# yassouali/pytorch-segmentation

Hardware: NVIDIA H100
Metric: images/sec DeepLabV3+/ResNet101 513x513 train step (fwd+CE+bwd+SGD) (higher is better)
Workload: dtype bf16

## Files before the change

include/seg_b200.h:

```cpp
#ifndef SEG_B200_H
#define SEG_B200_H

#include <stdint.h>

#ifdef __cplusplus
extern "C" {
#endif

#define SEG_DT_BF16 0
#define SEG_DT_F32 1

#define SEG_IMPL_AUTO 0
#define SEG_IMPL_SIMT 1
#define SEG_IMPL_TC 2

typedef struct seg_conv_desc {
  int32_t N, H, W, C;
  int32_t K;
  int32_t R, S;
  int32_t stride, pad, dil;
  int32_t P, Q;
  int32_t ldx;
  int32_t ldy;
} seg_conv_desc;

typedef struct seg_sync_desc {
  void* const* peers;
  int32_t rank, world, n_max;
  int64_t timeout_clocks;
  int32_t mode;
} seg_sync_desc;

const char* seg_last_error(void);
int seg_version(void);
int seg_device_ok(void);
int64_t seg_launch_count(void);
void seg_launch_count_reset(void);

int seg_conv2d_fwd(const seg_conv_desc* d, const void* x, const void* w_packed, void* y, int y_dtype,
                   const float* bias, float beta, double* stats, const seg_sync_desc* sync, void* sync_ticket,
                   int impl, void* stream);
int seg_conv2d_dgrad(const seg_conv_desc* d, const void* dy, const void* w_packed, void* dx, float beta,
                     int impl, void* stream);
int64_t seg_conv2d_wgrad_workspace_floats(const seg_conv_desc* d, int impl);
int seg_conv2d_wgrad(const seg_conv_desc* d, const void* dy, const void* x, float* dw_packed, float* workspace, int impl,
                     void* stream);

int64_t seg_dwconv_scratch_floats(int C);
int seg_dwconv3x3_fwd(const seg_conv_desc* d, const void* x, const float* w9, void* y, double* stats,
                      const seg_sync_desc* sync, void* sync_ticket, void* stream);
int seg_dwconv3x3_bwd_data(const seg_conv_desc* d, const void* dy, const float* w9, void* dx, float beta, void* stream);
int seg_dwconv3x3_bwd_weight(const seg_conv_desc* d, const void* dy, const void* x, float* dw9, float beta,
                             float* scratch, void* stream);
int seg_dw_pack_weight(const float* w_c133, float* w9, int C, void* stream);
int seg_dw_unpack_wgrad(const float* g9, float* g_c133, int C, float beta, void* stream);

int seg_pack_weight(const float* w_oihw, void* w_packed, int K, int C, int R, int S, int Cpad, void* stream);
int seg_unpack_wgrad(const float* dw_packed, float* g_oihw, int K, int C, int R, int S, int Cpad, float beta,
                     void* stream);
int seg_pack_entry_bytes(void);
int seg_pack_weights_batched(const void* table, int n, int64_t total, void* stream);
int seg_unpack_wgrads_batched(const void* table, int n, int64_t total, float beta, void* stream);
int seg_im2col(const seg_conv_desc* d, const void* x, int x_nchw_f32, void* col, int Kpad, void* stream);

int seg_bn_stats(const void* x, int64_t M, int C, int ldx, double* stats, const seg_sync_desc* sync, void* sync_ticket,
                 void* stream);
int seg_bn_finalize(const double* stats, double count, int C, const float* gamma, const float* beta, float eps,
                    float momentum, int clamp_eps, float* running_mean, float* running_var, float* scale_shift,
                    float* save_mean_istd, void* stream);
// ... 141 lines not shown
```

pytorch-segmentation_b200/csrc/seg_api.cu:

```cuda
#include <stdarg.h>
#include "seg_common.cuh"
#include "seg_sync.cuh"

namespace seg {

static thread_local char g_err[1024] = "";
std::atomic<long long> g_launches{0};

void set_error(const char* fmt, ...) {
  va_list ap;
  va_start(ap, fmt);
  vsnprintf(g_err, sizeof(g_err), fmt, ap);
  va_end(ap);
}

namespace tc {
bool supported(const seg_conv_desc* d);
int conv_fwd(const seg_conv_desc* d, const void* x, const void* w, void* y, int y_dtype, const float* bias, float beta,
             double* stats, unsigned* stat_ticket, const SyncDesc* sync, cudaStream_t stream);
int conv_dgrad(const seg_conv_desc* d, const void* dy, const void* w, void* dx, float beta, cudaStream_t stream);
int conv_wgrad(const seg_conv_desc* d, const void* dy, const void* x, float* dw, float* ws, cudaStream_t stream);
int64_t wgrad_workspace_floats(const seg_conv_desc* d);
}
namespace simt {
int conv_fwd(const seg_conv_desc* d, const void* x, const void* w, void* y, int y_dtype, const float* bias, float beta,
             double* stats, unsigned* stat_ticket, const seg_sync_desc* sync, cudaStream_t stream);
int conv_dgrad(const seg_conv_desc* d, const void* dy, const void* w, void* dx, float beta, cudaStream_t stream);
int conv_wgrad(const seg_conv_desc* d, const void* dy, const void* x, float* dw, cudaStream_t stream);
}

static int check_desc(const seg_conv_desc* d) {
  SEG_REQUIRE(d != nullptr, "null conv descriptor");
  SEG_REQUIRE(d->N > 0 && d->H > 0 && d->W > 0 && d->C > 0 && d->K > 0 && d->R > 0 && d->S > 0, "bad conv dims");
  SEG_REQUIRE(d->stride >= 1 && d->dil >= 1 && d->pad >= 0, "bad conv stride/dil/pad");
  const int P = (d->H + 2 * d->pad - d->dil * (d->R - 1) - 1) / d->stride + 1;
  const int Q = (d->W + 2 * d->pad - d->dil * (d->S - 1) - 1) / d->stride + 1;
  SEG_REQUIRE(P == d->P && Q == d->Q, "conv output size mismatch: expected %dx%d got %dx%d", P, Q, d->P, d->Q);
  SEG_REQUIRE(d->ldx >= d->C && d->ldy >= d->K, "conv pitch smaller than channel count");
  return 0;
}

static bool tma_base_ok(const void* p) { return (reinterpret_cast<uintptr_t>(p) & 15) == 0; }

}
// ... 40 lines not shown
    return tc::conv_fwd(d, x, w_packed, y, y_dtype, bias, beta, stats, tk, sync ? &sd : nullptr, ST(stream));
  }
  return simt::conv_fwd(d, x, w_packed, y, y_dtype, bias, beta, stats, tk, sync, ST(stream));
}

int seg_conv2d_dgrad(const seg_conv_desc* d, const void* dy, const void* w_packed, void* dx, float beta, int impl,
                     void* stream) {
  if (check_desc(d)) return 1;
  const bool tc_ok = tc::supported(d) && d->ldy % 8 == 0 && tma_base_ok(dy) && tma_base_ok(w_packed);
  if (impl == SEG_IMPL_TC || (impl == SEG_IMPL_AUTO && tc_ok))
    return tc::conv_dgrad(d, dy, w_packed, dx, beta, ST(stream));
  return simt::conv_dgrad(d, dy, w_packed, dx, beta, ST(stream));
}

static bool wgrad_on_tc(const seg_conv_desc* d, int impl) {
  return impl == SEG_IMPL_TC || (impl == SEG_IMPL_AUTO && tc::supported(d) && d->ldy % 8 == 0);
}

int64_t seg_conv2d_wgrad_workspace_floats(const seg_conv_desc* d, int impl) {
  if (check_desc(d)) return -1;
  return wgrad_on_tc(d, impl) ? tc::wgrad_workspace_floats(d) : 0;
}

int seg_conv2d_wgrad(const seg_conv_desc* d, const void* dy, const void* x, float* dw_packed, float* workspace, int impl,
                     void* stream) {
  if (check_desc(d)) return 1;
  if (wgrad_on_tc(d, impl) && (impl == SEG_IMPL_TC || (tma_base_ok(dy) && tma_base_ok(x))))
    return tc::conv_wgrad(d, dy, x, dw_packed, workspace, ST(stream));
  return simt::conv_wgrad(d, dy, x, dw_packed, ST(stream));
}

}
```

pytorch-segmentation_b200/csrc/seg_conv_tc.cu:

```cuda
#include <cuda.h>
#include <mutex>
#include <stdlib.h>
#include "seg_common.cuh"
#include "seg_ptx.cuh"
#include "seg_sync.cuh"

namespace seg {
namespace tc {

using namespace ptx;

constexpr int BM = 128;
constexpr int BK = 64;
constexpr int A_BYTES = BM * 128;
constexpr int KIND_KK = 0, KIND_KM = 1;
constexpr int NTHREADS = 384;
constexpr int NCONS = 256;
constexpr int MAXT = 49;

constexpr int BAR_CONSUMERS = 1;
constexpr int BAR_ORDER = 2;
constexpr int BAR_WG = 4;

struct TcParams {
// ... 3 lines not shown
  int Ncols;
  int taps;
  int kchunks;
  int stride;
  int lower_h, lower_w;
  int PQ, Q;
  int x_im2col;
  int brows_per_tap;
  short tap_wt[MAXT];
  short tap_oh[MAXT];
  short tap_ow[MAXT];
  void* out;
  long long ldo;
  int out_dtype;
  float beta;
  const float* bias;
  double* stats;
  int stat_rows;
  unsigned* stat_ticket;
  SyncDesc sync;
  int out_strided, out_H, out_W, osy, osx, opy, opx;
  int n_tiles, tiles;
  int kblocks_total, kblocks_per_split;
  float* dw;
  int dw_K, dw_C;
  float* ws;
};

__device__ __forceinline__ void row_to_coords(int m, int PQ, int Q, int stride, int lower_h, int lower_w, int& n, int& h,
                                              int& w) {
  n = m / PQ;
  int rem = m - n * PQ;
  int pp = rem / Q;
  int qq = rem - pp * Q;
  h = lower_h + pp * stride;
  w = lower_w + qq * stride;
}

template <int BN, int TA, int TB>
__device__ __forceinline__ void wgmma_tile(float* acc, uint64_t adesc, uint64_t bdesc, uint32_t accumulate) {
  if constexpr (BN == 64) wgmma_m64n64k16<TA, TB>(acc, adesc, bdesc, accumulate);
  else if constexpr (BN == 128) wgmma_m64n128k16<TA, TB>(acc, adesc, bdesc, accumulate);
  else wgmma_m64n256k16<TA, TB>(acc, adesc, bdesc, accumulate);
}

template <int BN, int KIND>
// ... 274 lines not shown

template <int BN>
struct Cfg {
  static constexpr int B_BYTES = BN * 128;
  static constexpr int STAGE_BYTES = A_BYTES + B_BYTES;
  static constexpr int STAGES = BN == 64 ? 6 : (BN == 128 ? 5 : 4);
  static constexpr int SMEM = STAGES * STAGE_BYTES + 1024  + 256 ;
  static_assert(STAGES * STAGE_BYTES >= BM * BN * 4, "staging tile must fit in the pipeline ring");
  static_assert(SMEM <= 227 * 1024, "shared memory per block");
};

template <int BN>
__global__ void __launch_bounds__(NTHREADS, 1) conv_gemm_wgrad(const __grid_constant__ TcParams p) {
  using C = Cfg<BN>;
  constexpr int STAGES = C::STAGES;
  extern __shared__ uint8_t smem_raw[];
  const uint32_t raw_addr = smem_u32(smem_raw);
  const uint32_t smem0 = (raw_addr + 1023u) & ~1023u;
  uint8_t* smem_gen = smem_raw + (smem0 - raw_addr);
  const uint32_t bar0 = smem0 + STAGES * C::STAGE_BYTES;
  auto full_bar = [&](int s) { return bar0 + 8u * s; };
  auto empty_bar = [&](int s) { return bar0 + 8u * (STAGES + s); };

  const int m0 = blockIdx.x * BM;
  const int n0 = blockIdx.y * BN;

  const int tap_mm = blockIdx.z % p.taps;
  const int split = blockIdx.z / p.taps;
  const int kb_begin = split * p.kblocks_per_split;
  const int kb_end = min(kb_begin + p.kblocks_per_split, p.kblocks_total);
  const int num_iters = max(kb_end - kb_begin, 0);

  if (threadIdx.x == 0) {
    prefetch_tmap(&p.mapA);
    prefetch_tmap(&p.mapB);
    for (int s = 0; s < STAGES; ++s) {
      mbar_init(full_bar(s), 1);
      mbar_init(empty_bar(s), 8);
    }
    fence_mbar_init();
  }
  __syncthreads();
  pdl_wait();

  if (threadIdx.x < 128) {
    if (threadIdx.x == 0 && num_iters > 0) {
      const uint16_t oh = (uint16_t)p.tap_oh[tap_mm], ow = (uint16_t)p.tap_ow[tap_mm];
      int it = 0;
      for (int kb = kb_begin; kb < kb_end; ++kb, ++it) {
        const int st = it % STAGES;
        const uint32_t ph = (it / STAGES) & 1;
        mbar_wait_nocall(empty_bar(st), ph ^ 1u);
        const uint32_t a_dst = smem0 + st * C::STAGE_BYTES;
        const uint32_t b_dst = a_dst + A_BYTES;
        const int pix0 = kb * BK;
        mbar_arrive_expect_tx(full_bar(st), C::STAGE_BYTES);
        tma_load_2d(a_dst, &p.mapA, full_bar(st), m0, pix0);
        tma_load_2d(a_dst + 8192, &p.mapA, full_bar(st), m0 + 64, pix0);
        if (p.x_im2col) {
          int n_img, h0, w0;
          row_to_coords(pix0, p.PQ, p.Q, p.stride, p.lower_h, p.lower_w, n_img, h0, w0);
#pragma unroll
          for (int j = 0; j < BN / 64; ++j)
            tma_load_im2col_4d(b_dst + j * 8192, &p.mapB, full_bar(st), n0 + j * 64, w0, h0, n_img, ow, oh);
        } else {
#pragma unroll
          for (int j = 0; j < BN / 64; ++j) tma_load_2d(b_dst + j * 8192, &p.mapB, full_bar(st), n0 + j * 64, pix0);
        }
      }
    }
    return;
  }

  if (num_iters == 0) return;
  const int ctid = threadIdx.x - 128;
  const int cw = ctid >> 7;
  const int warp = (ctid >> 5) & 3, lane = ctid & 31;
  float acc[BN / 2];
#pragma unroll
  for (int i = 0; i < BN / 2; ++i) acc[i] = 0.f;
  for (int it = 0; it < num_iters; ++it) {
    const int st = it % STAGES;
    mbar_wait_nocall(full_bar(st), (it / STAGES) & 1);
    const uint32_t a_addr = smem0 + st * C::STAGE_BYTES + cw * 8192;
    const uint32_t b_addr = smem0 + st * C::STAGE_BYTES + A_BYTES;
    const uint64_t adesc0 = make_smem_desc_sw128(a_addr, 8192, 1024);
    const uint64_t bdesc0 = make_smem_desc_sw128(b_addr, 8192, 1024);
    wgmma_fence();
#pragma unroll
    for (int k = 0; k < BK / 16; ++k)
      wgmma_tile<BN, 1, 1>(acc, adesc0 + (uint64_t)(k * 2048 >> 4), bdesc0 + (uint64_t)(k * 2048 >> 4), 1u);
    wgmma_commit();
    wgmma_wait<1>();
    __syncwarp();
    if (it > 0 && lane == 0) mbar_arrive(empty_bar((it - 1) % STAGES));
  }
  wgmma_wait<0>();
  named_sync(BAR_CONSUMERS, NCONS);

  uint8_t* stage = smem_gen;
  const int ncols_tile = min(BN, p.Ncols - n0);
  stage_acc<BN>(acc, nullptr, stage, cw * 64, warp, lane, nullptr, true);
  named_sync(BAR_CONSUMERS, NCONS);

  const int CPR = BN * 4 / 16;
  const int swz = (CPR >= 32 ? 31 : CPR - 1);
  float* base = p.ws ? p.ws + (size_t)split * p.taps * p.dw_K * p.dw_C : p.dw;
  for (int idx = ctid; idx < BM * CPR; idx += NCONS) {
    const int tr = idx / CPR, c16 = idx - tr * CPR;
    const int row = m0 + tr, col0 = c16 * 4;
    if (row >= p.M || col0 >= ncols_tile) continue;
    const float4 v = *reinterpret_cast<const float4*>(stage + (size_t)tr * (BN * 4) + ((c16 ^ (tr & swz)) << 4));
    float* dst = base + ((size_t)tap_mm * p.dw_K + row) * p.dw_C + n0 + col0;
    const bool vec = col0 + 4 <= ncols_tile && ((reinterpret_cast<uintptr_t>(dst) & 15) == 0);
    const float a[4] = {v.x, v.y, v.z, v.w};
    if (p.ws) {
      if (vec)
        *reinterpret_cast<float4*>(dst) = v;
      else
        for (int i = 0; i < 4; ++i)
          if (col0 + i < ncols_tile) dst[i] = a[i];
    } else if (vec) {
      asm volatile("red.global.add.v4.f32 [%0], {%1, %2, %3, %4};" ::"l"(dst), "f"(v.x), "f"(v.y), "f"(v.z), "f"(v.w)
                   : "memory");
    } else {
      for (int i = 0; i < 4; ++i)
        if (col0 + i < ncols_tile) atomicAdd(dst + i, a[i]);
    }
  }
}

typedef CUresult (*EncodeTiledFn)(CUtensorMap*, CUtensorMapDataType, cuuint32_t, void*, const cuuint64_t*,
                                  const cuuint64_t*, const cuuint32_t*, const cuuint32_t*, CUtensorMapInterleave,
                                  CUtensorMapSwizzle, CUtensorMapL2promotion, CUtensorMapFloatOOBfill);
typedef CUresult (*EncodeIm2colFn)(CUtensorMap*, CUtensorMapDataType, cuuint32_t, void*, const cuuint64_t*,
                                   const cuuint64_t*, const int*, const int*, cuuint32_t, cuuint32_t,
                                   const cuuint32_t*, CUtensorMapInterleave, CUtensorMapSwizzle,
                                   CUtensorMapL2promotion, CUtensorMapFloatOOBfill);
static EncodeTiledFn g_encode_tiled = nullptr;
static EncodeIm2colFn g_encode_im2col = nullptr;
static int g_driver_version = 0;

static int resolve_driver() {
  static std::once_flag once;
  static int status = 0;
  std::call_once(once, [] {
    void* f1 = nullptr;
    void* f2 = nullptr;
    cudaDriverEntryPointQueryResult q;
    if (cudaGetDriverEntryPoint("cuTensorMapEncodeTiled", &f1, cudaEnableDefault, &q) != cudaSuccess || !f1) status = 1;
    if (cudaGetDriverEntryPoint("cuTensorMapEncodeIm2col", &f2, cudaEnableDefault, &q) != cudaSuccess || !f2) status = 1;
// ... 252 lines not shown
    dw[i] += acc;
  }
}

static void wgrad_plan(const seg_conv_desc* d, int& bn, int& splits, int& kblocks_per_split) {
  const bool wide = d->R * d->S >= 9 && d->C >= 256 && d->C % 256 == 0;
  bn = (d->C <= 64) ? 64 : (wide ? 256 : 128);
  const int kblocks_total = (int)ceil_div64((int64_t)d->N * d->P * d->Q, BK);
  const int tiles = ceil_div(d->K, BM) * ceil_div(d->C, bn) * d->R * d->S;
  splits = max(1, num_sms() / tiles);
  splits = min(splits, kblocks_total);
  splits = min(splits, 1024);
  kblocks_per_split = ceil_div(kblocks_total, splits);
  splits = ceil_div(kblocks_total, kblocks_per_split);
}

int64_t wgrad_workspace_floats(const seg_conv_desc* d) {
  if (!supported(d)) return 0;
  int bn, splits, kps;
  wgrad_plan(d, bn, splits, kps);
  return splits > 1 ? (int64_t)splits * d->R * d->S * d->K * d->C : 0;
}

int conv_wgrad(const seg_conv_desc* d, const void* dy, const void* x, float* dw, float* ws, cudaStream_t stream) {
  SEG_REQUIRE(supported(d) && d->ldy % 8 == 0, "wgmma conv wgrad: unsupported shape");
  TcParams p;
  memset(&p, 0, sizeof(p));
  const int64_t npix = (int64_t)d->N * d->P * d->Q;
  SEG_REQUIRE(npix < (1ll << 31), "too many pixels");
  p.M = d->K;
  p.Ncols = d->C;
  p.taps = d->R * d->S;
  for (int t = 0; t < p.taps; ++t) {
    p.tap_wt[t] = (short)t;
    p.tap_oh[t] = (short)((t / d->S) * d->dil);
    p.tap_ow[t] = (short)((t % d->S) * d->dil);
  }
  p.stride = d->stride;
  p.lower_h = p.lower_w = -d->pad;
  p.PQ = d->P * d->Q;
  p.Q = d->Q;
  p.dw = dw;
  p.dw_K = d->K;
  p.dw_C = d->C;
  p.kblocks_total = (int)ceil_div64(npix, BK);
  int bn, splits;
  wgrad_plan(d, bn, splits, p.kblocks_per_split);
  SEG_REQUIRE(splits == 1 || ws != nullptr, "wgmma conv wgrad: %d k-splits need the workspace (seg_conv2d_wgrad_workspace_floats)", splits);
  SEG_REQUIRE((int64_t)(splits - 1) * p.kblocks_per_split < p.kblocks_total, "wgmma conv wgrad: split %d has no k-blocks", splits - 1);
  if (splits > 1) p.ws = ws;
  if (make_map_2d(&p.mapA, dy, npix, d->K, d->ldy, 64)) return 1;
  if (is_pointwise(d)) {
    p.x_im2col = 0;
    if (make_map_2d(&p.mapB, x, npix, d->C, d->ldx, 64)) return 1;
  } else {
    p.x_im2col = 1;
    const int upper = d->pad - (d->R - 1) * d->dil;
    if (make_map_im2col(&p.mapB, x, d->N, d->H, d->W, d->C, d->ldx, -d->pad, -d->pad, upper, upper, d->stride, 64)) return 1;
  }
  SEG_REQUIRE((unsigned)(p.taps * splits) <= 65535u, "wgrad grid.z too large");
  dim3 grid((unsigned)ceil_div(d->K, BM), (unsigned)ceil_div(d->C, bn), (unsigned)(p.taps * splits));
  if (launch_wgrad_bn(bn, p, grid, stream)) return 1;
  if (splits == 1) return 0;
  const int64_t n = (int64_t)p.taps * d->K * d->C;
  wgrad_split_reduce_kernel<<<(unsigned)std::min<int64_t>(ceil_div64(n, 256), (int64_t)num_sms() * 8), 256, 0, stream>>>(ws, splits, n, dw);
  return check_launch("wgrad_split_reduce");
}

}
}
```

pytorch-segmentation_b200/seg_b200/engine.py:

```python
import torch

from . import ops
from .lib import IMPL_AUTO

BN_EPS = 1e-5
BN_MOM = 0.1
FUSED_BWD_MAX_BYTES = 24 << 20
ACT_DTYPE = torch.bfloat16


class Act:
    __slots__ = ("t", "grad", "needs_grad", "_written")

    def __init__(self, t, needs_grad=True):
        self.t = t
        self.grad = None
        self.needs_grad = needs_grad
        self._written = False

    @property
    def shape(self):
        return self.t.shape

    def grad_target(self):
        if self.grad is None:
            self.grad = torch.empty(self.t.shape, dtype=ACT_DTYPE, device=self.t.device)
        if not self._written:
            self._written = True
            return self.grad, 0.0
        return self.grad, 1.0

# ... 68 lines not shown
                 step_ctr=None, arena_floats=0, owner=None):
        self.training = training
        self.record = training if record is None else record
        self.back = []
        self.back_params = {}
        self.grads = grads if grads is not None else {}
        self.touched = set()
        self.impl = impl
        self.dropout = dropout
        self.seed = seed
        self.sync = sync
        self.step_ctr = step_ctr
        self.packed_override = {}
        self.dw_buffers = {}
        self.clamp_eps = clamp_eps
        self._drop_ctr = 0
        self._pushed = set()
        self.bn_modules = []
        self.owner = owner
        self._arena_hint = int(arena_floats)
        self._arena = None
        self._arena_off = 0
        self.arena_used = 0

    def sync_active(self):
        s = self.sync
        return s is not None and (s.world > 1 or getattr(s, "force", False))

    def sync_fused(self):
        return self.sync_active() and getattr(self.sync, "fused", False)

    def zalloc(self, n, device):
        n_al = (int(n) + 31) // 32 * 32
        if self._arena is None or self._arena_off + n_al > self._arena.numel() or self._arena.device != device:
            size = max(self._arena_hint if self._arena is None else 0, n_al, 1 << 20)
            self._arena = torch.zeros(size, dtype=torch.float32, device=device)
            self._arena_off = 0
        v = self._arena[self._arena_off:self._arena_off + int(n)]
        self._arena_off += n_al
        self.arena_used += n_al
        return v

    def zalloc64(self, n, device):
        return self.zalloc(2 * int(n), device).view(torch.float64)

    def _param_grad(self, p, value_fn):
        if not p.requires_grad:
            return
        self.touched.add(p)
        if p in self.grads:
            value_fn(self.grads[p], 1.0)
        else:
            g = torch.empty(p.shape, dtype=torch.float32, device=p.device)
            value_fn(g, 0.0)
            self.grads[p] = g

    def _push_back(self, fn, params=()):
        if params:
            self.back_params[len(self.back)] = tuple(p for p in params if p is not None)
        self.back.append(fn)

    def backward(self, after=None):
        for i in range(len(self.back) - 1, -1, -1):
            self.back[i]()
            if after is not None:
                after(i)
        if self.owner is not None and self.arena_used:
            self.owner._arena_floats = self.arena_used
        self.back = []

    def conv(self, x, spec, out=None, out_dtype=None, want_stats=False):
        wp = self.packed_override.get(spec)
        if wp is None:
            wp = spec.packed()
        bias = spec.m.bias
        stats = None
        if out_dtype is None:
            out_dtype = ACT_DTYPE
        want = want_stats and self.training
        sync = tk = None
        if want:
            stats = self.zalloc64(2 * spec.K, wp.device)
            if self.sync_fused():
                sync, tk = self.sync, self.zalloc(1, wp.device)
        if spec.explicit:
            nchw = not isinstance(x, Act)
            src = x if nchw else x.t
            col = ops.im2col(src, spec.R, spec.S, spec.stride, spec.pad, spec.dil, spec.kpad, nchw_f32=nchw)
            y = ops.conv2d_fwd(col, wp, spec.K, 1, 1, out=out, out_dtype=out_dtype, bias=bias.detach() if bias is not None else None,
                               stats=stats, impl=self.impl, sync=sync, sync_ticket=tk)
            xin, geo = col, (1, 1, 1, 0, 1)
        else:
            y = ops.conv2d_fwd(x.t, wp, spec.K, spec.R, spec.S, spec.stride, spec.pad, spec.dil, out=out, out_dtype=out_dtype,
                               bias=bias.detach() if bias is not None else None, stats=stats, impl=self.impl, sync=sync, sync_ticket=tk)
            xin, geo = x.t, (spec.R, spec.S, spec.stride, spec.pad, spec.dil)
        ya = Act(y)
        if sync is not None:
            self._pushed.add(stats.data_ptr())
        if self.record:
            def bwd():
                dy = ya.grad
                if dy is None:
                    return
                R, S, stride, pad, dil = geo
                if spec.m.weight.requires_grad and spec in self.dw_buffers:
                    ops.conv2d_wgrad(dy, xin, R, S, stride, pad, dil, out=self.dw_buffers[spec], impl=self.impl)
                    self.touched.add(spec.m.weight)
                elif spec.m.weight.requires_grad:
                    dwp = ops.conv2d_wgrad(dy, xin, R, S, stride, pad, dil, impl=self.impl)
                    if spec.explicit:
                        def fill(g, beta):
                            full = dwp[0, :, : spec.R * spec.S * spec.C].reshape(spec.K, spec.R, spec.S, spec.C).permute(0, 3, 1, 2)
                            if beta:
                                g.add_(full)
                            else:
                                g.copy_(full)
                    else:
                        def fill(g, beta):
                            ops.unpack_wgrad(dwp, tuple(spec.m.weight.shape), beta=beta, out=g)
                    self._param_grad(spec.m.weight, fill)
                if bias is not None and bias.requires_grad:
                    cpad = ops.ld(dy)
                    wide = dy if dy.shape[-1] % 8 == 0 else dy.as_strided(dy.shape[:-1] + (cpad,), dy.stride(), dy.storage_offset())
                    s = ops.bn_stats(wide)[: spec.K].float()
                    self._param_grad(bias, lambda g, beta: g.add_(s) if beta else g.copy_(s))
                if (not spec.explicit) and isinstance(x, Act) and x.needs_grad:
                    gx, beta = x.grad_target()
                    ops.conv2d_dgrad(dy, wp, tuple(x.t.shape), R, S, stride, pad, dil, out=gx, beta=beta, impl=self.impl)
                ya.grad = None
            self._push_back(bwd, (spec.m.weight, bias))
        return ya, stats

    def dwconv(self, x, spec, want_stats=False):
        w9 = spec.packed()
        stats = self.zalloc64(2 * spec.C, w9.device) if (want_stats and self.training) else None
        sync = self.sync if (stats is not None and self.sync_fused()) else None
        y = ops.dwconv_fwd(x.t, w9, spec.stride, spec.pad, spec.dil, stats=stats, sync=sync,
                           sync_ticket=self.zalloc(1, w9.device) if sync is not None else None)
        if sync is not None:
            self._pushed.add(stats.data_ptr())
        ya = Act(y)
        if self.record:
            def bwd():
                dy = ya.grad
                if dy is None:
                    return
                if spec.m.weight.requires_grad:
                    g9 = ops.dwconv_bwd_weight(dy, x.t, spec.stride, spec.pad, spec.dil)
                    self._param_grad(spec.m.weight, lambda g, beta: ops.dw_unpack_wgrad(g9, g, beta))
                if x.needs_grad:
                    gx, beta = x.grad_target()
                    ops.dwconv_bwd_data(dy, w9, tuple(x.t.shape), spec.stride, spec.pad, spec.dil, out=gx, beta=beta)
                ya.grad = None
            self._push_back(bwd, (spec.m.weight,))
# ... 197 lines not shown
```

pytorch-segmentation_b200/seg_b200/lib.py:

```python
import ctypes
import os
from ctypes import POINTER, Structure, c_char_p, c_double, c_float, c_int, c_int32, c_int64, c_uint8, c_uint32, c_uint64, c_void_p

import torch

_HERE = os.path.dirname(os.path.abspath(__file__))
LIB_PATH = os.path.join(os.path.dirname(_HERE), "libseg_b200.so")

DT_BF16, DT_F32 = 0, 1
IMPL_AUTO, IMPL_SIMT, IMPL_TC = 0, 1, 2
LOSS_CE, LOSS_WCE, LOSS_FOCAL = 0, 1, 2


class SyncDesc(Structure):

    _fields_ = [("peers", c_void_p), ("rank", c_int32), ("world", c_int32), ("n_max", c_int32), ("timeout_clocks", c_int64),
                ("mode", c_int32)]


class ConvDesc(Structure):

    _fields_ = [(n, c_int32) for n in ("N", "H", "W", "C", "K", "R", "S", "stride", "pad", "dil", "P", "Q", "ldx", "ldy")]


def conv_out_size(size, k, stride, pad, dil):
    return (size + 2 * pad - dil * (k - 1) - 1) // stride + 1


def make_conv_desc(N, H, W, C, K, R, S, stride, pad, dil, ldx=None, ldy=None):
    P = conv_out_size(H, R, stride, pad, dil)
    Q = conv_out_size(W, S, stride, pad, dil)
    return ConvDesc(N, H, W, C, K, R, S, stride, pad, dil, P, Q, ldx if ldx is not None else C, ldy if ldy is not None else K)


_SIGS = {
    "seg_last_error": (c_char_p, []),
    "seg_version": (c_int, []),
    "seg_device_ok": (c_int, []),
    "seg_launch_count": (c_int64, []),
    "seg_launch_count_reset": (None, []),
    "seg_conv2d_fwd": (c_int, [POINTER(ConvDesc), c_void_p, c_void_p, c_void_p, c_int, c_void_p, c_float, c_void_p, c_void_p, c_void_p, c_int, c_void_p]),
    "seg_conv2d_dgrad": (c_int, [POINTER(ConvDesc), c_void_p, c_void_p, c_void_p, c_float, c_int, c_void_p]),
    "seg_conv2d_wgrad_workspace_floats": (c_int64, [POINTER(ConvDesc), c_int]),
    "seg_conv2d_wgrad": (c_int, [POINTER(ConvDesc), c_void_p, c_void_p, c_void_p, c_void_p, c_int, c_void_p]),
    "seg_dwconv_scratch_floats": (c_int64, [c_int]),
    "seg_dwconv3x3_fwd": (c_int, [POINTER(ConvDesc), c_void_p, c_void_p, c_void_p, c_void_p, c_void_p, c_void_p, c_void_p]),
    "seg_dwconv3x3_bwd_data": (c_int, [POINTER(ConvDesc), c_void_p, c_void_p, c_void_p, c_float, c_void_p]),
    "seg_dwconv3x3_bwd_weight": (c_int, [POINTER(ConvDesc), c_void_p, c_void_p, c_void_p, c_float, c_void_p, c_void_p]),
    "seg_dw_pack_weight": (c_int, [c_void_p, c_void_p, c_int, c_void_p]),
    "seg_dw_unpack_wgrad": (c_int, [c_void_p, c_void_p, c_int, c_float, c_void_p]),
    "seg_pack_weight": (c_int, [c_void_p, c_void_p, c_int, c_int, c_int, c_int, c_int, c_void_p]),
    "seg_unpack_wgrad": (c_int, [c_void_p, c_void_p, c_int, c_int, c_int, c_int, c_int, c_float, c_void_p]),
    "seg_pack_entry_bytes": (c_int, []),
    "seg_pack_weights_batched": (c_int, [c_void_p, c_int, c_int64, c_void_p]),
    "seg_unpack_wgrads_batched": (c_int, [c_void_p, c_int, c_int64, c_float, c_void_p]),
    "seg_im2col": (c_int, [POINTER(ConvDesc), c_void_p, c_int, c_void_p, c_int, c_void_p]),
    "seg_bn_stats": (c_int, [c_void_p, c_int64, c_int, c_int, c_void_p, c_void_p, c_void_p, c_void_p]),
    "seg_bn_finalize": (c_int, [c_void_p, c_double, c_int, c_void_p, c_void_p, c_float, c_float, c_int, c_void_p, c_void_p, c_void_p, c_void_p, c_void_p]),
    "seg_bn_eval_scale_shift": (c_int, [c_int, c_void_p, c_void_p, c_void_p, c_void_p, c_float, c_void_p, c_void_p, c_void_p]),
    "seg_bn_apply": (c_int, [c_void_p, c_int, c_void_p, c_void_p, c_int, c_void_p, c_int, c_int64, c_int, c_int, c_float, c_uint64, c_void_p, c_int, c_void_p]),
    "seg_counter_add": (c_int, [c_void_p, c_uint64, c_void_p]),
    "seg_bn_bwd_reduce_slots": (c_int, []),
    "seg_bn_bwd_reduce": (c_int, [c_void_p, c_int, c_void_p, c_int, c_void_p, c_int, c_void_p, c_int64, c_int, c_int, c_float, c_void_p, c_void_p, c_void_p, c_void_p, c_void_p, c_int, c_void_p, c_void_p, c_void_p, c_void_p]),
    "seg_bn_apply_train": (c_int, [c_void_p, c_int, c_void_p, c_double, c_void_p, c_void_p, c_float, c_float, c_int, c_void_p, c_void_p, c_void_p, c_void_p, c_int, c_void_p, c_int, c_int64, c_int, c_int, c_float, c_uint64, c_void_p, c_int, c_void_p, c_void_p, c_void_p]),
    "seg_bn_bwd_fused_workspace": (c_int, [c_int64, c_int, POINTER(c_int64), POINTER(c_int64)]),
    "seg_bn_bwd_fused": (c_int, [c_void_p, c_int, c_void_p, c_int, c_void_p, c_int, c_void_p, c_void_p, c_void_p, c_double, c_int64, c_int, c_int, c_float,
                                 c_void_p, c_void_p, c_void_p, c_void_p, c_void_p, c_int, c_void_p, c_int, c_void_p, c_int, c_float, c_int, c_void_p, c_void_p]),
# ... 113 lines not shown
```

pytorch-segmentation_b200/seg_b200/ops.py:

```python
import ctypes

import torch

from . import lib
from .lib import DT_BF16, DT_F32, IMPL_AUTO, IMPL_SIMT, IMPL_TC, ConvDesc, call, make_conv_desc, ptr

_IMPL_OVERRIDE = None
PROFILE = None


def _meta(d):
    if lib.TRACE is None:
        return None
    return (d.N, d.H, d.W, d.C, d.K, d.R, d.stride, d.dil, 2.0 * d.N * d.P * d.Q * d.K * d.C * d.R * d.S)


def _meta_rows(M, C, passes, flag=0):
    if lib.TRACE is None:
        return None
    return (int(M), int(C), int(flag), 0, 0, 0, 0, 0, 2.0 * M * C * passes)


def _prof(kind, d):
    if PROFILE is None:
# ... 84 lines not shown
    ev = _prof("fprop", d)
    call("seg_conv2d_fwd", ctypes.byref(d), ptr(x), ptr(w_packed), ptr(out), DT_BF16 if out.dtype == torch.bfloat16 else DT_F32,
         ptr(bias), float(beta), ptr(stats), sp, tp, _impl(impl), meta=_meta(d))
    if ev is not None:
        ev.record()
    return out


def conv2d_dgrad(dy, w_packed, x_shape, R, S, stride=1, pad=0, dil=1, out=None, beta=0.0, impl=IMPL_AUTO):
    N, H, W, C = x_shape
    K = dy.shape[-1]
    if out is None:
        out = torch.empty((N, H, W, C), dtype=torch.bfloat16, device=dy.device)
        beta = 0.0
    d = make_conv_desc(N, H, W, C, K, R, S, stride, pad, dil, ldx=ld(out), ldy=ld(dy))
    assert (d.P, d.Q) == (dy.shape[1], dy.shape[2])
    ev = _prof("dgrad", d)
    call("seg_conv2d_dgrad", ctypes.byref(d), ptr(dy), ptr(w_packed), ptr(out), float(beta), _impl(impl), meta=_meta(d))
    if ev is not None:
        ev.record()
    return out


def conv2d_wgrad(dy, x, R, S, stride=1, pad=0, dil=1, out=None, impl=IMPL_AUTO):
    N, H, W, C = x.shape
    K = dy.shape[-1]
    if out is None:
        out = torch.zeros((R * S, K, C), dtype=torch.float32, device=x.device)
    d = make_conv_desc(N, H, W, C, K, R, S, stride, pad, dil, ldx=ld(x), ldy=ld(dy))
    assert (d.P, d.Q) == (dy.shape[1], dy.shape[2])
    nws = lib.load().seg_conv2d_wgrad_workspace_floats(ctypes.byref(d), _impl(impl))
    if nws < 0:
        raise RuntimeError(f"seg_conv2d_wgrad_workspace_floats failed: {lib.last_error()}")
    ws = torch.empty(nws, dtype=torch.float32, device=x.device) if nws > 0 else None
    ev = _prof("wgrad", d)
    call("seg_conv2d_wgrad", ctypes.byref(d), ptr(dy), ptr(x), ptr(out), ptr(ws), _impl(impl), meta=_meta(d))
    if ev is not None:
        ev.record()
    return out


def dw_pack_weight(w_c133):
    C = w_c133.shape[0]
    w9 = torch.empty((9, C), dtype=torch.float32, device=w_c133.device)
    call("seg_dw_pack_weight", ptr(w_c133), ptr(w9), C)
    return w9


def dw_unpack_wgrad(g9, out, beta=0.0):
    call("seg_dw_unpack_wgrad", ptr(g9), ptr(out), g9.shape[1], float(beta))
    return out


def _dw_desc(x_shape, stride, pad, dil, ldx, ldy):
    N, H, W, C = x_shape
    return make_conv_desc(N, H, W, C, C, 3, 3, stride, pad, dil, ldx=ldx, ldy=ldy)


def dwconv_fwd(x, w9, stride=1, pad=1, dil=1, out=None, stats=None, sync=None, sync_ticket=None):
# ... 433 lines not shown
```

pytorch-segmentation_b200/seg_b200/train.py:

```python
import numpy as np
import torch
import torch.distributed as dist

from . import lib, ops
from . import metrics as _metrics
from .engine import Tape


class WeightTables:

    def __init__(self, model, grad_views, dev):
        specs = [s for s in model.all_conv_specs()]
        self.specs = specs
        for ds in model.all_dw_specs():
            ds.always_repack = True
        dt = np.dtype([("oihw", "<u8"), ("packed", "<u8"), ("K", "<i4"), ("C", "<i4"), ("R", "<i4"), ("S", "<i4"),
                       ("Cpad", "<i4"), ("explicit", "<i4"), ("start", "<i8")])
        assert dt.itemsize == lib.load().seg_pack_entry_bytes()
        want_g = grad_views is not None
        n_dw = sum(int(np.prod(s.packed_shape())) for s in specs if s.m.weight.requires_grad) if want_g else 0
        self.flat_dwp = torch.zeros(n_dw, dtype=torch.float32, device=dev)
        pack = np.zeros(len(specs), dtype=dt)
        unp = []
        self.packed_bufs, self.dw_bufs = {}, {}
# ... 248 lines not shown
        g = torch.cuda.CUDAGraph()
        if self.world > 1:
            dist.barrier()
        with torch.cuda.graph(g, capture_error_mode="thread_local" if self.world > 1 else "global"):
            loss = self._step_impl(xs, ys)
        self.steps -= 1
        self._graph, self._static = g, (xs, ys, loss)

    def _backward_bucketed(self, tape):
        last = {}
        for i, ps in tape.back_params.items():
            for p in ps:
                b = self.bucket_of.get(p)
                if b is not None and (b not in last or i < last[b]):
                    last[b] = i
        fire = {}
        for b, i in last.items():
            fire.setdefault(i, []).append(b)
        cur = torch.cuda.current_stream()
        done = set()

        def launch(b):
            done.add(b)
            tab = self.sub_unpack.get(b)
            if tab is not None:
                lib.call("seg_unpack_wgrads_batched", tab[0].data_ptr(), tab[1], tab[2], 0.0)
            ev = torch.cuda.Event()
            ev.record(cur)
            lo, hi = self.buckets[b]
            with torch.cuda.stream(self.side):
                self.side.wait_event(ev)
                dist.all_reduce(self.flat_grad[lo:hi])

        def after(i):
            for b in sorted(fire.get(i, ()), reverse=True):
                launch(b)

        tape.backward(after=after)
        for b in range(len(self.buckets) - 1, -1, -1):
            if b not in done:
                launch(b)
        cur.wait_stream(self.side)

    def _step_impl(self, x, target):
        m = self.model
        self.flat_grad.zero_()
        self.wt.zero_wgrads()
        self.wt.pack()
        tape = m._new_tape(True, True)
        tape.grads = dict(self.grad_views)
        tape.packed_override, tape.dw_buffers = self.wt.packed_bufs, self.wt.dw_bufs
        heads = m._forward_heads(tape, x.contiguous().float())
        total = None
        spec = self.loss_spec
# ... 24 lines not shown
```

Before: 299.0.

## Run conv weight-gradients on a side stream and make wgrad kernel persistent

Conv weight-gradient and bias-gradient work now goes to a dedicated side stream, so it can overlap with the data-gradient chain on the main stream. The stream joins at the end of backward, and the bucketed allreduce path waits on a wgrad event before unpacking and reducing. The TC wgrad kernel becomes a grid-stride loop over work items with an optional CTA cap, keeping the mbarrier phase continuous across items, though the default cap of zero still launches one CTA per item. This adds cross-stream event overhead and the risk of contention between the two streams.

```diff
diff --git a/include/seg_b200.h b/include/seg_b200.h
--- a/include/seg_b200.h
+++ b/include/seg_b200.h
@@ -45,6 +45,8 @@
 int64_t seg_conv2d_wgrad_workspace_floats(const seg_conv_desc* d, int impl);
 int seg_conv2d_wgrad(const seg_conv_desc* d, const void* dy, const void* x, float* dw_packed, float* workspace, int impl,
                      void* stream);
+int seg_conv2d_wgrad_ctas(const seg_conv_desc* d, const void* dy, const void* x, float* dw_packed, float* workspace,
+                          int impl, int max_ctas, void* stream);
 
 int64_t seg_dwconv_scratch_floats(int C);
 int seg_dwconv3x3_fwd(const seg_conv_desc* d, const void* x, const float* w9, void* y, double* stats,
diff --git a/pytorch-segmentation_b200/csrc/seg_api.cu b/pytorch-segmentation_b200/csrc/seg_api.cu
--- a/pytorch-segmentation_b200/csrc/seg_api.cu
+++ b/pytorch-segmentation_b200/csrc/seg_api.cu
@@ -19,7 +19,8 @@
 int conv_fwd(const seg_conv_desc* d, const void* x, const void* w, void* y, int y_dtype, const float* bias, float beta,
              double* stats, unsigned* stat_ticket, const SyncDesc* sync, cudaStream_t stream);
 int conv_dgrad(const seg_conv_desc* d, const void* dy, const void* w, void* dx, float beta, cudaStream_t stream);
-int conv_wgrad(const seg_conv_desc* d, const void* dy, const void* x, float* dw, float* ws, cudaStream_t stream);
+int conv_wgrad(const seg_conv_desc* d, const void* dy, const void* x, float* dw, float* ws, int max_ctas,
+               cudaStream_t stream);
 int64_t wgrad_workspace_floats(const seg_conv_desc* d);
 }
 namespace simt {
@@ -106,12 +107,21 @@
   return wgrad_on_tc(d, impl) ? tc::wgrad_workspace_floats(d) : 0;
 }
 
-int seg_conv2d_wgrad(const seg_conv_desc* d, const void* dy, const void* x, float* dw_packed, float* workspace, int impl,
-                     void* stream) {
+int seg_conv2d_wgrad_ctas(const seg_conv_desc* d, const void* dy, const void* x, float* dw_packed, float* workspace,
+                          int impl, int max_ctas, void* stream) {
   if (check_desc(d)) return 1;
+  if (max_ctas < 0) {
+    set_error("seg_conv2d_wgrad_ctas: max_ctas = %d < 0", max_ctas);
+    return 1;
+  }
   if (wgrad_on_tc(d, impl) && (impl == SEG_IMPL_TC || (tma_base_ok(dy) && tma_base_ok(x))))
-    return tc::conv_wgrad(d, dy, x, dw_packed, workspace, ST(stream));
+    return tc::conv_wgrad(d, dy, x, dw_packed, workspace, max_ctas, ST(stream));
   return simt::conv_wgrad(d, dy, x, dw_packed, ST(stream));
 }
 
+int seg_conv2d_wgrad(const seg_conv_desc* d, const void* dy, const void* x, float* dw_packed, float* workspace, int impl,
+                     void* stream) {
+  return seg_conv2d_wgrad_ctas(d, dy, x, dw_packed, workspace, impl, 0, stream);
 }
+
+}
diff --git a/pytorch-segmentation_b200/csrc/seg_conv_tc.cu b/pytorch-segmentation_b200/csrc/seg_conv_tc.cu
--- a/pytorch-segmentation_b200/csrc/seg_conv_tc.cu
+++ b/pytorch-segmentation_b200/csrc/seg_conv_tc.cu
@@ -49,6 +49,7 @@
   int out_strided, out_H, out_W, osy, osx, opy, opx;
   int n_tiles, tiles;
   int kblocks_total, kblocks_per_split;
+  int wg_mt, wg_nt, wg_items;
   float* dw;
   int dw_K, dw_C;
   float* ws;
@@ -369,15 +370,6 @@
   auto full_bar = [&](int s) { return bar0 + 8u * s; };
   auto empty_bar = [&](int s) { return bar0 + 8u * (STAGES + s); };
 
-  const int m0 = blockIdx.x * BM;
-  const int n0 = blockIdx.y * BN;
-
-  const int tap_mm = blockIdx.z % p.taps;
-  const int split = blockIdx.z / p.taps;
-  const int kb_begin = split * p.kblocks_per_split;
-  const int kb_end = min(kb_begin + p.kblocks_per_split, p.kblocks_total);
-  const int num_iters = max(kb_end - kb_begin, 0);
-
   if (threadIdx.x == 0) {
     prefetch_tmap(&p.mapA);
     prefetch_tmap(&p.mapB);
@@ -390,90 +382,106 @@
   __syncthreads();
   pdl_wait();
 
-  if (threadIdx.x < 128) {
-    if (threadIdx.x == 0 && num_iters > 0) {
-      const uint16_t oh = (uint16_t)p.tap_oh[tap_mm], ow = (uint16_t)p.tap_ow[tap_mm];
-      int it = 0;
-      for (int kb = kb_begin; kb < kb_end; ++kb, ++it) {
-        const int st = it % STAGES;
-        const uint32_t ph = (it / STAGES) & 1;
-        mbar_wait_nocall(empty_bar(st), ph ^ 1u);
-        const uint32_t a_dst = smem0 + st * C::STAGE_BYTES;
-        const uint32_t b_dst = a_dst + A_BYTES;
-        const int pix0 = kb * BK;
-        mbar_arrive_expect_tx(full_bar(st), C::STAGE_BYTES);
-        tma_load_2d(a_dst, &p.mapA, full_bar(st), m0, pix0);
-        tma_load_2d(a_dst + 8192, &p.mapA, full_bar(st), m0 + 64, pix0);
-        if (p.x_im2col) {
-          int n_img, h0, w0;
-          row_to_coords(pix0, p.PQ, p.Q, p.stride, p.lower_h, p.lower_w, n_img, h0, w0);
-#pragma unroll
-          for (int j = 0; j < BN / 64; ++j)
-            tma_load_im2col_4d(b_dst + j * 8192, &p.mapB, full_bar(st), n0 + j * 64, w0, h0, n_img, ow, oh);
-        } else {
-#pragma unroll
-          for (int j = 0; j < BN / 64; ++j) tma_load_2d(b_dst + j * 8192, &p.mapB, full_bar(st), n0 + j * 64, pix0);
-        }
-      }
-    }
-    return;
-  }
-
-  if (num_iters == 0) return;
   const int ctid = threadIdx.x - 128;
   const int cw = ctid >> 7;
   const int warp = (ctid >> 5) & 3, lane = ctid & 31;
-  float acc[BN / 2];
-#pragma unroll
-  for (int i = 0; i < BN / 2; ++i) acc[i] = 0.f;
-  for (int it = 0; it < num_iters; ++it) {
-    const int st = it % STAGES;
-    mbar_wait_nocall(full_bar(st), (it / STAGES) & 1);
-    const uint32_t a_addr = smem0 + st * C::STAGE_BYTES + cw * 8192;
-    const uint32_t b_addr = smem0 + st * C::STAGE_BYTES + A_BYTES;
-    const uint64_t adesc0 = make_smem_desc_sw128(a_addr, 8192, 1024);
-    const uint64_t bdesc0 = make_smem_desc_sw128(b_addr, 8192, 1024);
-    wgmma_fence();
-#pragma unroll
-    for (int k = 0; k < BK / 16; ++k)
-      wgmma_tile<BN, 1, 1>(acc, adesc0 + (uint64_t)(k * 2048 >> 4), bdesc0 + (uint64_t)(k * 2048 >> 4), 1u);
-    wgmma_commit();
-    wgmma_wait<1>();
-    __syncwarp();
-    if (it > 0 && lane == 0) mbar_arrive(empty_bar((it - 1) % STAGES));
-  }
-  wgmma_wait<0>();
-  named_sync(BAR_CONSUMERS, NCONS);
-
-  uint8_t* stage = smem_gen;
-  const int ncols_tile = min(BN, p.Ncols - n0);
-  stage_acc<BN>(acc, nullptr, stage, cw * 64, warp, lane, nullptr, true);
-  named_sync(BAR_CONSUMERS, NCONS);
-
-  const int CPR = BN * 4 / 16;
-  const int swz = (CPR >= 32 ? 31 : CPR - 1);
-  float* base = p.ws ? p.ws + (size_t)split * p.taps * p.dw_K * p.dw_C : p.dw;
-  for (int idx = ctid; idx < BM * CPR; idx += NCONS) {
-    const int tr = idx / CPR, c16 = idx - tr * CPR;
-    const int row = m0 + tr, col0 = c16 * 4;
-    if (row >= p.M || col0 >= ncols_tile) continue;
-    const float4 v = *reinterpret_cast<const float4*>(stage + (size_t)tr * (BN * 4) + ((c16 ^ (tr & swz)) << 4));
-    float* dst = base + ((size_t)tap_mm * p.dw_K + row) * p.dw_C + n0 + col0;
-    const bool vec = col0 + 4 <= ncols_tile && ((reinterpret_cast<uintptr_t>(dst) & 15) == 0);
-    const float a[4] = {v.x, v.y, v.z, v.w};
-    if (p.ws) {
-      if (vec)
-        *reinterpret_cast<float4*>(dst) = v;
-      else
-        for (int i = 0; i < 4; ++i)
-          if (col0 + i < ncols_tile) dst[i] = a[i];
-    } else if (vec) {
-      asm volatile("red.global.add.v4.f32 [%0], {%1, %2, %3, %4};" ::"l"(dst), "f"(v.x), "f"(v.y), "f"(v.z), "f"(v.w)
-                   : "memory");
-    } else {
-      for (int i = 0; i < 4; ++i)
-        if (col0 + i < ncols_tile) atomicAdd(dst + i, a[i]);
-    }
+  int base = 0;
+  for (int item = blockIdx.x; item < p.wg_items; item += gridDim.x) {
+    const int m0 = (item % p.wg_mt) * BM;
+    const int n0 = ((item / p.wg_mt) % p.wg_nt) * BN;
+    const int z = item / (p.wg_mt * p.wg_nt);
+
+    const int tap_mm = z % p.taps;
+    const int split = z / p.taps;
+    const int kb_begin = split * p.kblocks_per_split;
+    const int kb_end = min(kb_begin + p.kblocks_per_split, p.kblocks_total);
+    const int num_iters = max(kb_end - kb_begin, 0);
+
+    if (threadIdx.x < 128) {
+      if (threadIdx.x == 0 && num_iters > 0) {
+        const uint16_t oh = (uint16_t)p.tap_oh[tap_mm], ow = (uint16_t)p.tap_ow[tap_mm];
+        int it = base;
+        for (int kb = kb_begin; kb < kb_end; ++kb, ++it) {
+          const int st = it % STAGES;
+          const uint32_t ph = (it / STAGES) & 1;
+          mbar_wait_nocall(empty_bar(st), ph ^ 1u);
+          const uint32_t a_dst = smem0 + st * C::STAGE_BYTES;
+          const uint32_t b_dst = a_dst + A_BYTES;
+          const int pix0 = kb * BK;
+          mbar_arrive_expect_tx(full_bar(st), C::STAGE_BYTES);
+          tma_load_2d(a_dst, &p.mapA, full_bar(st), m0, pix0);
+          tma_load_2d(a_dst + 8192, &p.mapA, full_bar(st), m0 + 64, pix0);
+          if (p.x_im2col) {
+            int n_img, h0, w0;
+            row_to_coords(pix0, p.PQ, p.Q, p.stride, p.lower_h, p.lower_w, n_img, h0, w0);
+#pragma unroll
+            for (int j = 0; j < BN / 64; ++j)
+              tma_load_im2col_4d(b_dst + j * 8192, &p.mapB, full_bar(st), n0 + j * 64, w0, h0, n_img, ow, oh);
+          } else {
+#pragma unroll
+            for (int j = 0; j < BN / 64; ++j) tma_load_2d(b_dst + j * 8192, &p.mapB, full_bar(st), n0 + j * 64, pix0);
+          }
+        }
+      }
+    } else if (num_iters > 0) {
+      float acc[BN / 2];
+#pragma unroll
+      for (int i = 0; i < BN / 2; ++i) acc[i] = 0.f;
+      for (int it = 0; it < num_iters; ++it) {
+        const int g = base + it;
+        const int st = g % STAGES;
+        mbar_wait_nocall(full_bar(st), (g / STAGES) & 1);
+        const uint32_t a_addr = smem0 + st * C::STAGE_BYTES + cw * 8192;
+        const uint32_t b_addr = smem0 + st * C::STAGE_BYTES + A_BYTES;
+        const uint64_t adesc0 = make_smem_desc_sw128(a_addr, 8192, 1024);
+        const uint64_t bdesc0 = make_smem_desc_sw128(b_addr, 8192, 1024);
+        wgmma_fence();
+#pragma unroll
+        for (int k = 0; k < BK / 16; ++k)
+          wgmma_tile<BN, 1, 1>(acc, adesc0 + (uint64_t)(k * 2048 >> 4), bdesc0 + (uint64_t)(k * 2048 >> 4), 1u);
+        wgmma_commit();
+        wgmma_wait<1>();
+        __syncwarp();
+        if (it > 0 && lane == 0) mbar_arrive(empty_bar((g - 1) % STAGES));
+      }
+      wgmma_wait<0>();
+      __syncwarp();
+      if (lane == 0) mbar_arrive(empty_bar((base + num_iters - 1) % STAGES));
+      named_sync(BAR_CONSUMERS, NCONS);
+
+      uint8_t* stage = smem_gen;
+      const int ncols_tile = min(BN, p.Ncols - n0);
+      stage_acc<BN>(acc, nullptr, stage, cw * 64, warp, lane, nullptr, true);
+      named_sync(BAR_CONSUMERS, NCONS);
+
+      const int CPR = BN * 4 / 16;
+      const int swz = (CPR >= 32 ? 31 : CPR - 1);
+      float* out = p.ws ? p.ws + (size_t)split * p.taps * p.dw_K * p.dw_C : p.dw;
+      for (int idx = ctid; idx < BM * CPR; idx += NCONS) {
+        const int tr = idx / CPR, c16 = idx - tr * CPR;
+        const int row = m0 + tr, col0 = c16 * 4;
+        if (row >= p.M || col0 >= ncols_tile) continue;
+        const float4 v = *reinterpret_cast<const float4*>(stage + (size_t)tr * (BN * 4) + ((c16 ^ (tr & swz)) << 4));
+        float* dst = out + ((size_t)tap_mm * p.dw_K + row) * p.dw_C + n0 + col0;
+        const bool vec = col0 + 4 <= ncols_tile && ((reinterpret_cast<uintptr_t>(dst) & 15) == 0);
+        const float a[4] = {v.x, v.y, v.z, v.w};
+        if (p.ws) {
+          if (vec)
+            *reinterpret_cast<float4*>(dst) = v;
+          else
+            for (int i = 0; i < 4; ++i)
+              if (col0 + i < ncols_tile) dst[i] = a[i];
+        } else if (vec) {
+          asm volatile("red.global.add.v4.f32 [%0], {%1, %2, %3, %4};" ::"l"(dst), "f"(v.x), "f"(v.y), "f"(v.z), "f"(v.w)
+                       : "memory");
+        } else {
+          for (int i = 0; i < 4; ++i)
+            if (col0 + i < ncols_tile) atomicAdd(dst + i, a[i]);
+        }
+      }
+    }
+    base += num_iters;
+    __syncthreads();
   }
 }
 
@@ -772,7 +780,8 @@
   return splits > 1 ? (int64_t)splits * d->R * d->S * d->K * d->C : 0;
 }
 
-int conv_wgrad(const seg_conv_desc* d, const void* dy, const void* x, float* dw, float* ws, cudaStream_t stream) {
+int conv_wgrad(const seg_conv_desc* d, const void* dy, const void* x, float* dw, float* ws, int max_ctas,
+               cudaStream_t stream) {
   SEG_REQUIRE(supported(d) && d->ldy % 8 == 0, "wgmma conv wgrad: unsupported shape");
   TcParams p;
   memset(&p, 0, sizeof(p));
@@ -808,9 +817,13 @@
     const int upper = d->pad - (d->R - 1) * d->dil;
     if (make_map_im2col(&p.mapB, x, d->N, d->H, d->W, d->C, d->ldx, -d->pad, -d->pad, upper, upper, d->stride, 64)) return 1;
   }
-  SEG_REQUIRE((unsigned)(p.taps * splits) <= 65535u, "wgrad grid.z too large");
-  dim3 grid((unsigned)ceil_div(d->K, BM), (unsigned)ceil_div(d->C, bn), (unsigned)(p.taps * splits));
-  if (launch_wgrad_bn(bn, p, grid, stream)) return 1;
+  p.wg_mt = ceil_div(d->K, BM);
+  p.wg_nt = ceil_div(d->C, bn);
+  const int64_t items = (int64_t)p.wg_mt * p.wg_nt * p.taps * splits;
+  SEG_REQUIRE(items < (1ll << 31), "wgrad: too many work items");
+  p.wg_items = (int)items;
+  const int ctas = max_ctas > 0 ? (int)std::min<int64_t>(items, max_ctas) : p.wg_items;
+  if (launch_wgrad_bn(bn, p, dim3((unsigned)ctas), stream)) return 1;
   if (splits == 1) return 0;
   const int64_t n = (int64_t)p.taps * d->K * d->C;
   wgrad_split_reduce_kernel<<<(unsigned)std::min<int64_t>(ceil_div64(n, 256), (int64_t)num_sms() * 8), 256, 0, stream>>>(ws, splits, n, dw);
diff --git a/pytorch-segmentation_b200/seg_b200/engine.py b/pytorch-segmentation_b200/seg_b200/engine.py
--- a/pytorch-segmentation_b200/seg_b200/engine.py
+++ b/pytorch-segmentation_b200/seg_b200/engine.py
@@ -7,6 +7,15 @@
 BN_MOM = 0.1
 FUSED_BWD_MAX_BYTES = 24 << 20
 ACT_DTYPE = torch.bfloat16
+
+_WGRAD_STREAMS = {}
+
+
+def _wgrad_stream(device):
+    s = _WGRAD_STREAMS.get(device)
+    if s is None:
+        s = _WGRAD_STREAMS[device] = torch.cuda.Stream(device)
+    return s
 
 
 class Act:
@@ -121,6 +130,32 @@
         self._arena = None
         self._arena_off = 0
         self.arena_used = 0
+        self._wg_stream = None
+        self._wg_hold = []
+
+    def _wg_fork(self, *reads):
+        if not reads[0].is_cuda:
+            return None
+        cur = torch.cuda.current_stream(reads[0].device)
+        if self._wg_stream is None:
+            self._wg_stream = _wgrad_stream(reads[0].device)
+        ev = torch.cuda.Event()
+        ev.record(cur)
+        self._wg_stream.wait_event(ev)
+        self._wg_hold.extend(reads)
+        return torch.cuda.stream(self._wg_stream)
+
+    def wgrad_event(self):
+        if self._wg_stream is None:
+            return None
+        ev = torch.cuda.Event()
+        ev.record(self._wg_stream)
+        return ev
+
+    def wgrad_join(self):
+        if self._wg_stream is not None:
+            torch.cuda.current_stream(self._wg_stream.device).wait_stream(self._wg_stream)
+        self._wg_hold = []
 
     def sync_active(self):
         s = self.sync
@@ -164,6 +199,7 @@
             self.back[i]()
             if after is not None:
                 after(i)
+        self.wgrad_join()
         if self.owner is not None and self.arena_used:
             self.owner._arena_floats = self.arena_used
         self.back = []
@@ -202,33 +238,44 @@
                 if dy is None:
                     return
                 R, S, stride, pad, dil = geo
-                if spec.m.weight.requires_grad and spec in self.dw_buffers:
-                    ops.conv2d_wgrad(dy, xin, R, S, stride, pad, dil, out=self.dw_buffers[spec], impl=self.impl)
-                    self.touched.add(spec.m.weight)
-                elif spec.m.weight.requires_grad:
-                    dwp = ops.conv2d_wgrad(dy, xin, R, S, stride, pad, dil, impl=self.impl)
-                    if spec.explicit:
-                        def fill(g, beta):
-                            full = dwp[0, :, : spec.R * spec.S * spec.C].reshape(spec.K, spec.R, spec.S, spec.C).permute(0, 3, 1, 2)
-                            if beta:
-                                g.add_(full)
-                            else:
-                                g.copy_(full)
-                    else:
-                        def fill(g, beta):
-                            ops.unpack_wgrad(dwp, tuple(spec.m.weight.shape), beta=beta, out=g)
-                    self._param_grad(spec.m.weight, fill)
-                if bias is not None and bias.requires_grad:
-                    cpad = ops.ld(dy)
-                    wide = dy if dy.shape[-1] % 8 == 0 else dy.as_strided(dy.shape[:-1] + (cpad,), dy.stride(), dy.storage_offset())
-                    s = ops.bn_stats(wide)[: spec.K].float()
-                    self._param_grad(bias, lambda g, beta: g.add_(s) if beta else g.copy_(s))
+                want_w = spec.m.weight.requires_grad
+                want_b = bias is not None and bias.requires_grad
+                side = self._wg_fork(dy, xin) if (want_w or want_b) else None
                 if (not spec.explicit) and isinstance(x, Act) and x.needs_grad:
                     gx, beta = x.grad_target()
                     ops.conv2d_dgrad(dy, wp, tuple(x.t.shape), R, S, stride, pad, dil, out=gx, beta=beta, impl=self.impl)
                 ya.grad = None
+                if side is None:
+                    self._conv_param_grads(spec, dy, xin, geo, want_w, want_b)
+                else:
+                    with side:
+                        self._conv_param_grads(spec, dy, xin, geo, want_w, want_b)
             self._push_back(bwd, (spec.m.weight, bias))
         return ya, stats
+
+    def _conv_param_grads(self, spec, dy, xin, geo, want_w, want_b):
+        R, S, stride, pad, dil = geo
+        if want_w and spec in self.dw_buffers:
+            ops.conv2d_wgrad(dy, xin, R, S, stride, pad, dil, out=self.dw_buffers[spec], impl=self.impl)
+            self.touched.add(spec.m.weight)
+        elif want_w:
+            dwp = ops.conv2d_wgrad(dy, xin, R, S, stride, pad, dil, impl=self.impl)
+            if spec.explicit:
+                def fill(g, beta):
+                    full = dwp[0, :, : spec.R * spec.S * spec.C].reshape(spec.K, spec.R, spec.S, spec.C).permute(0, 3, 1, 2)
+                    if beta:
+                        g.add_(full)
+                    else:
+                        g.copy_(full)
+            else:
+                def fill(g, beta):
+                    ops.unpack_wgrad(dwp, tuple(spec.m.weight.shape), beta=beta, out=g)
+            self._param_grad(spec.m.weight, fill)
+        if want_b:
+            cpad = ops.ld(dy)
+            wide = dy if dy.shape[-1] % 8 == 0 else dy.as_strided(dy.shape[:-1] + (cpad,), dy.stride(), dy.storage_offset())
+            s = ops.bn_stats(wide)[: spec.K].float()
+            self._param_grad(spec.m.bias, lambda g, beta: g.add_(s) if beta else g.copy_(s))
 
     def dwconv(self, x, spec, want_stats=False):
         w9 = spec.packed()
diff --git a/pytorch-segmentation_b200/seg_b200/lib.py b/pytorch-segmentation_b200/seg_b200/lib.py
--- a/pytorch-segmentation_b200/seg_b200/lib.py
+++ b/pytorch-segmentation_b200/seg_b200/lib.py
@@ -43,6 +43,7 @@
     "seg_conv2d_dgrad": (c_int, [POINTER(ConvDesc), c_void_p, c_void_p, c_void_p, c_float, c_int, c_void_p]),
     "seg_conv2d_wgrad_workspace_floats": (c_int64, [POINTER(ConvDesc), c_int]),
     "seg_conv2d_wgrad": (c_int, [POINTER(ConvDesc), c_void_p, c_void_p, c_void_p, c_void_p, c_int, c_void_p]),
+    "seg_conv2d_wgrad_ctas": (c_int, [POINTER(ConvDesc), c_void_p, c_void_p, c_void_p, c_void_p, c_int, c_int, c_void_p]),
     "seg_dwconv_scratch_floats": (c_int64, [c_int]),
     "seg_dwconv3x3_fwd": (c_int, [POINTER(ConvDesc), c_void_p, c_void_p, c_void_p, c_void_p, c_void_p, c_void_p, c_void_p]),
     "seg_dwconv3x3_bwd_data": (c_int, [POINTER(ConvDesc), c_void_p, c_void_p, c_void_p, c_float, c_void_p]),
diff --git a/pytorch-segmentation_b200/seg_b200/ops.py b/pytorch-segmentation_b200/seg_b200/ops.py
--- a/pytorch-segmentation_b200/seg_b200/ops.py
+++ b/pytorch-segmentation_b200/seg_b200/ops.py
@@ -130,7 +130,7 @@
     return out
 
 
-def conv2d_wgrad(dy, x, R, S, stride=1, pad=0, dil=1, out=None, impl=IMPL_AUTO):
+def conv2d_wgrad(dy, x, R, S, stride=1, pad=0, dil=1, out=None, impl=IMPL_AUTO, max_ctas=0):
     N, H, W, C = x.shape
     K = dy.shape[-1]
     if out is None:
@@ -142,7 +142,7 @@
         raise RuntimeError(f"seg_conv2d_wgrad_workspace_floats failed: {lib.last_error()}")
     ws = torch.empty(nws, dtype=torch.float32, device=x.device) if nws > 0 else None
     ev = _prof("wgrad", d)
-    call("seg_conv2d_wgrad", ctypes.byref(d), ptr(dy), ptr(x), ptr(out), ptr(ws), _impl(impl), meta=_meta(d))
+    call("seg_conv2d_wgrad_ctas", ctypes.byref(d), ptr(dy), ptr(x), ptr(out), ptr(ws), _impl(impl), int(max_ctas), meta=_meta(d))
     if ev is not None:
         ev.record()
     return out
diff --git a/pytorch-segmentation_b200/seg_b200/train.py b/pytorch-segmentation_b200/seg_b200/train.py
--- a/pytorch-segmentation_b200/seg_b200/train.py
+++ b/pytorch-segmentation_b200/seg_b200/train.py
@@ -294,14 +294,17 @@
 
         def launch(b):
             done.add(b)
-            tab = self.sub_unpack.get(b)
-            if tab is not None:
-                lib.call("seg_unpack_wgrads_batched", tab[0].data_ptr(), tab[1], tab[2], 0.0)
             ev = torch.cuda.Event()
             ev.record(cur)
+            wev = tape.wgrad_event()
             lo, hi = self.buckets[b]
             with torch.cuda.stream(self.side):
                 self.side.wait_event(ev)
+                if wev is not None:
+                    self.side.wait_event(wev)
+                tab = self.sub_unpack.get(b)
+                if tab is not None:
+                    lib.call("seg_unpack_wgrads_batched", tab[0].data_ptr(), tab[1], tab[2], 0.0)
                 dist.all_reduce(self.flat_grad[lo:hi])
 
         def after(i):
```

After: 306.6 (median of 6 runs). 2.5% higher.
